# zwpku/colvars-finder

Measured on AMD Instinct MI355X. Metric: MD frames/sec through EigenFunctionTask train step, higher is better.
Workload: dtype f32

## Files before the change

colvars-finder_amd/csrc/ef16_front.hip:

```cpp
#include "ef16_common.hpp"
#include "cvf_p2p.hpp"

namespace {
template <int H, int NH, int NIT, bool ALLAL>
__global__ __launch_bounds__(1024, 4) void ef16_front_kernel(cvf_mlp_desc mlp, const float* __restrict__ theta,
                                                             const float* __restrict__ packed, cvf_pp_desc pp,
                                                             const float* __restrict__ x, int64_t B,
                                                             const float* __restrict__ a, const float* __restrict__ w,
                                                             float* __restrict__ feat_tiled, float* __restrict__ y_tiled,
                                                             float* __restrict__ saved, float* __restrict__ q_tiled,
                                                             float* __restrict__ e_tiled, double* __restrict__ partial, int launch,
                                                             const float* __restrict__ x_lag, int64_t units_x,
                                                             const float* __restrict__ w_lag) {
  constexpr int RT = Hid<H>::RT, NG = Hid<H>::NG, SMAX = 18, CTMAX = 5;
  constexpr bool kTransfer = NIT == 0;
  extern __shared__ __attribute__((aligned(16))) float lds_all[];
  const int upb = launch & 0xff;
  const int k = mlp.n_nets, D = mlp.dims[0];
  const int wave_b = __builtin_amdgcn_readfirstlane((int)threadIdx.x >> 6);
  const int usub = upb > 1 ? wave_b / k : 0;
  const int wave = wave_b - usub * k;
  const int tid = (int)threadIdx.x - usub * (64 * k), lane_in = tid & 63;
  const int nthreads = upb > 1 ? 64 * k : (int)blockDim.x, nw = nthreads >> 6;
  const int net = wave;
  const int64_t ublock = (int64_t)blockIdx.x * upb + usub;
  const bool paired = kTransfer && x_lag != nullptr && (launch >> 8) != 0;
  const int nc = pp.n_coord, nal = pp.n_align, N = pp.n_rec;
  const int stride = x_tile_stride(nc);
  const Front16Lds Lo = front16_lds(nc, nal, k);
  float* lds = lds_all + usub * (kTransfer ? Lo.g + 16 : Lo.total);
  const int64_t n_ublock = (kTransfer && !paired) ? 2 * units_x : units_x;
  const int64_t ub = ublock < n_ublock ? ublock : n_ublock - 1;
  const float* const x_first = x;
  const float* const w_first = w;
  auto run_pass = [&](const int pass) __attribute__((always_inline)) {
  const int lane = lane_in;
  const PackLayout L = pack_layout(H, NH, D);
  const URows pk = urows(packed + (int64_t)net * L.per_net, L.per_net, lane);
  const int S = (D + 3) >> 2, CT = (D + 15) >> 4;
  float a0[SMAX][RT];
  float bias[NH][RT][4];
  const int q_ = lane >> 4;
  auto request_layer0 = [&]() {
#pragma unroll
    for (int s = 0; s < SMAX; ++s) {
      const int se = s < S ? s : S - 1;
#pragma unroll
      for (int rt = 0; rt < RT; ++rt) a0[s][rt] = pk.ld(L.f0() + (se * RT + rt) * 64);
    }
    load_hid_const_u<H>(urows(theta + mlp.b_off[net][0], H, q_), bias[0]);
  };
  const bool lagged = x_lag != nullptr && (paired ? pass == 1 : ub >= units_x);
  const int64_t unit = (lagged && !paired) ? ub - units_x : ub;
  const int64_t tile = (unit >> 2) + (lagged ? (units_x >> 2) : 0);
  const int sub = (int)(unit & 3);
  x = lagged ? x_lag : x_first;
  w = lagged ? w_lag : w_first;
  float* xt = lds;
  float* refL = lds + Lo.ref;
  float* aL = lds + Lo.a;
  float* auxL = lds + Lo.aux;
  float* wL = (kTransfer && pass == 1) ? lds + Lo.g : lds + Lo.w;
  float* rsL = lds + Lo.rs;
  float* yL = lds + Lo.y + (kTransfer ? pass * (k * kU) : 0);
  float* eL = lds + Lo.e;
  float* featI = lds + Lo.feat;
  float* gI = lds + Lo.g + net * (kU * kImgP);
  const int f = lane >> 2, p = lane & 3;
  const int col = lane & 15, q = lane >> 4;

  CVF_STAMP(20);
  if (stride == nc && (unit + 1) * kU <= B && (reinterpret_cast<uintptr_t>(x) & 15) == 0) {
    const float4* src = reinterpret_cast<const float4*>(x + unit * (int64_t)(kU * nc));
    float4* dst = reinterpret_cast<float4*>(xt);
    const int n4 = (kU * nc) >> 2;
    for (int v = tid; v < n4; v += nthreads) dst[v] = src[v];
  } else {
    load_x_tile<6>(x, B, nc, unit, xt, tid, nthreads, kU);
  }
  for (int j = tid; j < 3 * nal + nc; j += nthreads) refL[j] = j < 3 * nal ? pp.ref_c[j] : (a != nullptr ? a[j - 3 * nal] : 0.0f);
  if (tid < kU) {
    const int64_t frame = unit * kU + tid;
    wL[tid] = (w != nullptr && frame < B) ? w[frame] : 0.0f;
  }
  if (wave != 0) request_layer0();
  __syncthreads();
  const float* my = xt + f * stride;
  CVF_STAMP(21);

  if (wave == 0) {
    double acc[15];
#pragma unroll
    for (int i = 0; i < 15; ++i) acc[i] = 0.0;
#pragma unroll 2
    for (int b = p; b < nal; b += 4) {
      const double x0 = (double)my[3 * b], x1 = (double)my[3 * b + 1], x2 = (double)my[3 * b + 2];
      const double r0 = (double)refL[3 * b], r1 = (double)refL[3 * b + 1], r2 = (double)refL[3 * b + 2];
      acc[0] += x0; acc[1] += x1; acc[2] += x2;
      acc[3] = fma(x0, r0, acc[3]); acc[4] = fma(x0, r1, acc[4]); acc[5] = fma(x0, r2, acc[5]);
      acc[6] = fma(x1, r0, acc[6]); acc[7] = fma(x1, r1, acc[7]); acc[8] = fma(x1, r2, acc[8]);
      acc[9] = fma(x2, r0, acc[9]); acc[10] = fma(x2, r1, acc[10]); acc[11] = fma(x2, r2, acc[11]);
      acc[12] += r0; acc[13] += r1; acc[14] += r2;
    }
#pragma unroll
    for (int i = 0; i < 15; ++i) acc[i] = quad_sumd16(acc[i]);
    const double inv = fast_rcp((double)nal);
    const double cd[3] = {acc[0] * inv, acc[1] * inv, acc[2] * inv};
    double Hm[3][3];
#pragma unroll
    for (int i = 0; i < 3; ++i)
#pragma unroll
      for (int j = 0; j < 3; ++j) Hm[i][j] = fma(-cd[i], acc[12 + j], acc[3 + 3 * i + j]);
    KabschOut ko;
    if constexpr (kTransfer) {
      kabsch_from_H<false>(Hm, ko);
#pragma unroll
      for (int i = 0; i < 6; ++i) ko.Kinv[i] = 0.0f;
    } else {
      kabsch_from_H<true>(Hm, ko);
    }
    const Centre c = centre_of(cd);
    const float av[kAuxP] = {ko.R[0], ko.R[1], ko.R[2], ko.R[3], ko.R[4], ko.R[5], ko.R[6], ko.R[7], ko.R[8], c.hi[0], c.hi[1], c.hi[2],
                             ko.Kinv[0], ko.Kinv[1], ko.Kinv[2], ko.Kinv[3], ko.Kinv[4], ko.Kinv[5], c.lo[0], c.lo[1], c.lo[2]};
#pragma unroll
    for (int i = 0; i < kAuxP; ++i)
      if ((i & 3) == p) auxL[f * kAuxP + i] = av[i];
    if (lane < 3) rsL[lane] = (float)(lane == 0 ? acc[12] : lane == 1 ? acc[13] : acc[14]);
    request_layer0();
  }
  lds_barrier();
  CVF_STAMP(22);

  {
    float R[9];
    const float* ar = auxL + f * kAuxP;
#pragma unroll
    for (int i = 0; i < 9; ++i) R[i] = ar[i];
    Centre c;
#pragma unroll
    for (int i = 0; i < 3; ++i) {
      c.hi[i] = ar[9 + i];
      c.lo[i] = ar[18 + i];
    }
    for (int at = p + 4 * wave; at < N; at += 4 * nw) {
      const V3 al = row_times(centred(my, at, c), R);
      float* fi = featI + f * kImgP + 3 * at;
      fi[0] = al.x;
      fi[1] = al.y;
      fi[2] = al.z;
    }
  }
  lds_barrier();
  CVF_STAMP(23);

  Vec<H, 1> h[NH];
  auto set_bias = [&](Vec<H, 1>& X, const float (&b)[RT][4]) {
#pragma unroll
    for (int rt = 0; rt < RT; ++rt)
#pragma unroll
      for (int r = 0; r < 4; ++r) X.v[rt][0][r] = b[rt][r];
  };
  set_bias(h[0], bias[0]);
  {
    float bf[SMAX];
    const float* fr = featI + col * kImgP;
#pragma unroll
    for (int s = 0; s < SMAX; ++s) {
      const int kf = 4 * (s < S ? s : S - 1) + q;
      bf[s] = fr[kf < D ? kf : D - 1];
    }
    HFrag<H> hf[NH > 1 ? NH - 1 : 1];
#pragma unroll
    for (int l = 1; l < NH; ++l) {
      load_hfrag_u<H>(hf[l - 1], pk, L.fh(l));
      load_hid_const_u<H>(urows(theta + mlp.b_off[net][l], H, q), bias[l]);
    }
#pragma unroll
    for (int s = 0; s < SMAX; ++s) {
      if (s < S) {
#pragma unroll
        for (int rt = 0; rt < RT; ++rt) h[0].v[rt][0] = mfma4(a0[s][rt], bf[s], h[0].v[rt][0]);
      }
    }
    CVF_STAMP(24);
    tanh_inplace<H, 1>(h[0]);
#pragma unroll
    for (int l = 1; l < NH; ++l) {
      set_bias(h[l], bias[l]);
      hidden_mul<H, 1>(h[l], hf[l - 1], h[l - 1]);
      tanh_inplace<H, 1>(h[l]);
    }
  }
  float wl[RT][4];
  load_hid_const_u<H>(urows(theta + mlp.w_off[net][NH], H, q), wl);
  const float bL = theta[mlp.b_off[net][NH]];
  HFrag<H> tf[NH > 1 ? NH - 1 : 1];
#pragma unroll
  for (int l = 1; l < NH; ++l) load_hfrag_u<H>(tf[l - 1], pk, L.th(l));

  const URows sv = urows(saved + (tile * k + net) * (int64_t)(kHand<NH>() * NG * 256) + sub * 64, kHand<NH>() * NG * 256 - sub * 64, lane);
  {
    float part = 0.0f;
#pragma unroll
    for (int rt = 0; rt < RT; ++rt)
#pragma unroll
      for (int r = 0; r < 4; ++r) part = fmaf(wl[rt][r], h[NH - 1].v[rt][0][r], part);
    const float yv = sum_over_q(part) + bL;
    yL[net * kU + col] = yv;
    y_tiled[(tile * k + net) * CVF_TILE + kU * sub + col] = yv;
  }
  CVF_STAMP(25);
  if constexpr (kTransfer) {
#pragma unroll
    for (int l = 0; l < NH; ++l)
#pragma unroll
      for (int g = 0; g < NG; ++g) sv.st((l * NG + g) * 256, h[l].v[g >> 2][0][g & 3]);
    float* ft = feat_tiled + tile * (int64_t)D * CVF_TILE + kU * sub + f;
    const float* fi = featI + f * kImgP;
#pragma unroll 1
    for (int j = p + 4 * wave; j < D; j += 4 * nw) ft[j * CVF_TILE] = fi[j];
    return;
  } else {

  {
    float t0[CTMAX][NG];
#pragma unroll
    for (int rt = 0; rt < CTMAX; ++rt)
#pragma unroll
      for (int s = 0; s < NG; ++s) t0[rt][s] = pk.ld(L.t0() + ((rt < CT ? rt : CT - 1) * NG + s) * 64);
    Vec<H, 1> d;
#pragma unroll
    for (int rt = 0; rt < RT; ++rt)
#pragma unroll
      for (int r = 0; r < 4; ++r) {
        const float hv = h[NH - 1].v[rt][0][r];
        d.v[rt][0][r] = wl[rt][r] * (1.0f - hv * hv);
      }
    Vec<H, 1> ev[NH > 1 ? NH - 1 : 1];
#pragma unroll
    for (int l = NH - 1; l >= 1; --l) {
      init_bias<H, 1>(ev[l - 1], nullptr, q);
      hidden_mul<H, 1>(ev[l - 1], tf[l - 1], d);
      tangent_of<H, 1>(d, h[l - 1], ev[l - 1]);
    }
#pragma unroll
    for (int rt = 0; rt < CTMAX; ++rt) {
      if (rt < CT) {
        f32x4 acc = {0.0f, 0.0f, 0.0f, 0.0f};
#pragma unroll
        for (int s = 0; s < NG; ++s) acc = mfma4(t0[rt][s], d.v[s >> 2][0][s & 3], acc);
        if (16 * rt + 4 * q < D) *reinterpret_cast<float4*>(gI + col * kImgP + 16 * rt + 4 * q) = float4{acc[0], acc[1], acc[2], acc[3]};
      }
    }
#pragma unroll
    for (int l = 0; l < NH; ++l)
#pragma unroll
      for (int g = 0; g < NG; ++g) sv.st((l * NG + g) * 256, h[l].v[g >> 2][0][g & 3]);
#pragma unroll
    for (int l = 1; l < NH; ++l)
#pragma unroll
      for (int g = 0; g < NG; ++g) sv.st(((NH + l - 1) * NG + g) * 256, ev[l - 1].v[g >> 2][0][g & 3]);
  }
  CVF_STAMP(26);
  asm volatile("s_waitcnt lgkmcnt(0)" ::: "memory");

  float f0b[SMAX][RT];
  {
    float R[9];
    const float* ar = auxL + f * kAuxP;
#pragma unroll
    for (int i = 0; i < 9; ++i) R[i] = ar[i];
    const Centre c = centre_of(ar[9], ar[10], ar[11]);
    float* Ul = gI + f * kImgP;
    V3 gv[NIT];
    V3 gsum = v3(0.0f, 0.0f, 0.0f);
    Outer3 Mo = {{{0.0f, 0.0f}, {0.0f, 0.0f}, {0.0f, 0.0f}}, {0.0f, 0.0f, 0.0f}};
#pragma unroll
    for (int it = 0; it < NIT; ++it) {
      int at = p + 4 * it;
      asm volatile("" : "+v"(at));
      const bool last = it == NIT - 1;
      const int ac = (last && at >= N) ? N - 1 : at;
      const float lv = (last && at >= N) ? 0.0f : 1.0f;
      gv[it] = v3(Ul[3 * ac], Ul[3 * ac + 1], Ul[3 * ac + 2]);
      const V3 gm = last ? lv * gv[it] : gv[it];
      gsum = gsum + gm;
      outer_acc(Mo, centred(my, ac, c), gm);
    }
    CVF_STAMP(27);
    gsum = v3(quad_sumf16(gsum.x), quad_sumf16(gsum.y), quad_sumf16(gsum.z));
    const V3 sump = mat_times(R, gsum);
    float M[9];
    outer_to_array(Mo, M);
#pragma unroll
    for (int i = 0; i < 9; ++i) M[i] = quad_sumf16(M[i]);
    float T[9], Z[9];
#pragma unroll
    for (int i = 0; i < 3; ++i)
#pragma unroll
      for (int j = 0; j < 3; ++j) T[3 * i + j] = R[i] * M[j] + R[3 + i] * M[3 + j] + R[6 + i] * M[6 + j];
    float Kinv[6];
#pragma unroll
    for (int i = 0; i < 6; ++i) Kinv[i] = ar[12 + i];
    const V3 s = sym_times(Kinv, v3(T[7] - T[5], T[2] - T[6], T[3] - T[1]));
#pragma unroll
    for (int i = 0; i < 3; ++i) {
      Z[3 * i + 0] = R[3 * i + 1] * s.z - R[3 * i + 2] * s.y;
      Z[3 * i + 1] = -R[3 * i + 0] * s.z + R[3 * i + 2] * s.x;
      Z[3 * i + 2] = R[3 * i + 0] * s.y - R[3 * i + 1] * s.x;
    }
    const float inv_nal = 1.0f / (float)nal;
    const V3 shift = inv_nal * sump;
    const MatCols Rc = mat_cols(R), Zc = mat_cols(Z);
    f2 E2 = {0.0f, 0.0f};
    float Ez = 0.0f;
    f2 usum_xy = {0.0f, 0.0f};
    float usum_z = 0.0f;
    Outer3 dHo = {{{0.0f, 0.0f}, {0.0f, 0.0f}, {0.0f, 0.0f}}, {0.0f, 0.0f, 0.0f}};
#pragma unroll
    for (int it = 0; it < NIT; ++it) {
      int at = p + 4 * it;
      asm volatile("" : "+v"(at));
      const bool last = it == NIT - 1;
      const int ac = (last && at >= N) ? N - 1 : at;
      const float lv = (last && at >= N) ? 0.0f : 1.0f;
      const float ma = ALLAL ? 1.0f : (ac < nal ? 1.0f : 0.0f);
      const int ar_ = ALLAL ? ac : (ac < nal ? ac : 0);
      V3 rf = v3(refL[3 * ar_], refL[3 * ar_ + 1], refL[3 * ar_ + 2]);
      if (!ALLAL) rf = ma * rf;
      f2 Gxy = ALLAL ? f2{-shift.x, -shift.y} : f2{-ma * shift.x, -ma * shift.y};
      float Gz = ALLAL ? -shift.z : -ma * shift.z;
      mat_times_acc(Rc, gv[it], Gxy, Gz);
      mat_times_acc(Zc, rf, Gxy, Gz);
      const f2 uxy = f2{aL[3 * ac], aL[3 * ac + 1]} * Gxy;
      const float uz = aL[3 * ac + 2] * Gz;
      gv[it] = v3(uxy.x, uxy.y, uz);
      const bool masked = last || !ALLAL;
      const float m = ma * lv;
      const f2 uxm = masked ? m * uxy : uxy;
      const float uzm = masked ? m * uz : uz;
      E2 = fma2(last ? lv * uxy : uxy, Gxy, E2);
      Ez = fmaf(last ? lv * uz : uz, Gz, Ez);
      usum_xy += uxm; usum_z += uzm;
      outer_acc(dHo, v3(uxm.x, uxm.y, uzm), rf);
    }
    CVF_STAMP(28);
    const float E = quad_sumf16((E2.x + E2.y) + Ez);
    const V3 usum = v3(quad_sumf16(usum_xy.x), quad_sumf16(usum_xy.y), quad_sumf16(usum_z));
    const V3 rsum = v3(rsL[0], rsL[1], rsL[2]);
    float dH[9];
    outer_to_array(dHo, dH);
#pragma unroll
    for (int i = 0; i < 9; ++i) dH[i] = quad_sumf16(dH[i]);
    eL[net * kU + f] = E;
    e_tiled[(tile * k + net) * CVF_TILE + kU * sub + f] = E;
    const V3 ubar = inv_nal * usum;
    dH[0] -= ubar.x * rsum.x; dH[1] -= ubar.x * rsum.y; dH[2] -= ubar.x * rsum.z;
    dH[3] -= ubar.y * rsum.x; dH[4] -= ubar.y * rsum.y; dH[5] -= ubar.y * rsum.z;
    dH[6] -= ubar.z * rsum.x; dH[7] -= ubar.z * rsum.y; dH[8] -= ubar.z * rsum.z;
#pragma unroll
    for (int i = 0; i < 3; ++i)
#pragma unroll
      for (int j = 0; j < 3; ++j) T[3 * i + j] = R[i] * dH[j] + R[3 + i] * dH[3 + j] + R[6 + i] * dH[6 + j];
    asm volatile("" ::: "memory");
#pragma unroll
    for (int i = 0; i < 6; ++i) Kinv[i] = ar[12 + i];
    const V3 om = sym_times(Kinv, v3(T[7] - T[5], T[2] - T[6], T[3] - T[1]));
    float dR[9];
#pragma unroll
    for (int i = 0; i < 3; ++i) {
      dR[3 * i + 0] = R[3 * i + 1] * om.z - R[3 * i + 2] * om.y;
      dR[3 * i + 1] = -R[3 * i + 0] * om.z + R[3 * i + 2] * om.x;
      dR[3 * i + 2] = R[3 * i + 0] * om.y - R[3 * i + 1] * om.x;
    }
    CVF_STAMP(31);
    const MatRows Rr = mat_rows(R), dRr = mat_rows(dR);
#pragma unroll
    for (int it = 0; it < NIT; ++it) {
      int at = p + 4 * it;
      asm volatile("" : "+v"(at));
      const int ac = (it == NIT - 1 && at >= N) ? N - 1 : at;
      f2 qxy = {0.0f, 0.0f};
      float qz = 0.0f;
      row_times_acc(Rr, gv[it] - ubar, qxy, qz);
      row_times_acc(dRr, centred(my, ac, c), qxy, qz);
      gv[it] = v3(qxy.x, qxy.y, qz);
      Ul[3 * ac] = qxy.x;
      Ul[3 * ac + 1] = qxy.y;
      Ul[3 * ac + 2] = qz;
    }
    CVF_STAMP(32);
    asm volatile("" ::: "memory");
#pragma unroll
    for (int s_ = 0; s_ < SMAX; ++s_) {
      const int se = s_ < S ? s_ : S - 1;
#pragma unroll
      for (int rt = 0; rt < RT; ++rt) f0b[s_][rt] = pk.ld(L.f0() + (se * RT + rt) * 64);
    }
    {
      asm volatile("s_waitcnt lgkmcnt(0)" ::: "memory");
      Vec<H, 1> sv0;
      init_bias<H, 1>(sv0, nullptr, q);
      const float* qr = gI + col * kImgP;
#pragma unroll
      for (int s = 0; s < SMAX; ++s) {
        if (s < S) {
          const int kf = 4 * s + q;
          const float b = qr[kf < D ? kf : D - 1];
#pragma unroll
          for (int rt = 0; rt < RT; ++rt) sv0.v[rt][0] = mfma4(f0b[s][rt], b, sv0.v[rt][0]);
        }
      }
#pragma unroll
      for (int g = 0; g < NG; ++g) sv.st(((2 * NH - 1) * NG + g) * 256, sv0.v[g >> 2][0][g & 3]);
    }
    CVF_STAMP(33);
    float* qt = q_tiled + (tile * k + net) * (int64_t)D * CVF_TILE + kU * sub + f;
#pragma unroll
    for (int it = 0; it < NIT; ++it) {
      int at = p + 4 * it;
      asm volatile("" : "+v"(at));
      const int ac = (it == NIT - 1 && at >= N) ? N - 1 : at;
      qt[(3 * ac) * CVF_TILE] = gv[it].x;
      qt[(3 * ac + 1) * CVF_TILE] = gv[it].y;
      qt[(3 * ac + 2) * CVF_TILE] = gv[it].z;
    }
  }
  CVF_STAMP(34);
  {
    float* ft = feat_tiled + tile * (int64_t)D * CVF_TILE + kU * sub + f;
    const float* fi = featI + f * kImgP;
#pragma unroll 1
    for (int j = p + 4 * wave; j < D; j += 4 * nw) ft[j * CVF_TILE] = fi[j];
  }
  CVF_STAMP(29);
  if (partial == nullptr) return;
  lds_barrier();

  if (wave == 0) {
    typedef double f64x4 __attribute__((ext_vector_type(4)));
    const int np = CVF_NPAIR(k);
    const int i = lane & 15, kq = lane >> 4;
    f64x4 d1 = {0.0, 0.0, 0.0, 0.0}, d2 = {0.0, 0.0, 0.0, 0.0};
    const float* yrow = yL + (i >= 1 && i <= k ? i - 1 : 0) * kU;
    const float* erow = eL + (i < k ? i : 0) * kU;
#pragma unroll
    for (int s_ = 0; s_ < 4; ++s_) {
      const int fr = 4 * s_ + kq;
      const double wb = (double)wL[fr];
      const double yv = (double)yrow[fr];
      const double a1 = i == 0 ? 1.0 : (i <= k ? yv : 0.0);
      const double b = i == 0 ? wb : (i <= k ? wb * yv : 0.0);
      const double a2 = i < k ? (double)erow[fr] : 0.0;
      d1 = __builtin_amdgcn_mfma_f64_16x16x4f64(a1, b, d1, 0, 0, 0);
      d2 = __builtin_amdgcn_mfma_f64_16x16x4f64(a2, b, d2, 0, 0, 0);
    }
    const int cj = lane & 15;
    const int64_t G = units_x;
#pragma unroll
    for (int r = 0; r < 4; ++r) {
      const int ri = (lane >> 4) + 4 * r;
      int t = -1;
      if (ri == 0 && cj <= k) t = cj;
      else if (ri >= 1 && ri <= cj && cj <= k) {
        const int a_ = ri - 1, b_ = cj - 1;
        t = 1 + k + a_ * k - (a_ * (a_ - 1)) / 2 + (b_ - a_);
      }
      if (t >= 0) partial[t * G + unit] = d1[r];
      if (cj == 0 && ri < k) partial[(1 + k + np + ri) * G + unit] = d2[r];
    }
  }
  CVF_STAMP(30);
  }
  };
  run_pass(0);
  if constexpr (kTransfer) {
    if (!paired) return;
    run_pass(1);
    if (partial == nullptr) return;
    const int lane = lane_in;
    const int64_t unit = ub;
    lds_barrier();
    if (wave == 0) {
      typedef double f64x4 __attribute__((ext_vector_type(4)));
      const int np = CVF_NPAIR(k);
      const int i = lane & 15, kq = lane >> 4;
      const float* y0 = lds + Lo.y;
      const float* y1 = y0 + k * kU;
      const float* w0 = lds + Lo.w;
      const float* w1 = lds + Lo.g;
      f64x4 d1 = {0.0, 0.0, 0.0, 0.0}, d2 = {0.0, 0.0, 0.0, 0.0}, d3 = {0.0, 0.0, 0.0, 0.0};
      const int yi = (i >= 1 && i <= k ? i - 1 : 0) * kU, ti = (i < k ? i : 0) * kU;
#pragma unroll
      for (int s_ = 0; s_ < 4; ++s_) {
        const int fr = 4 * s_ + kq;
        const double wb = (double)w0[fr], wl_ = (double)w1[fr];
        const double yv = (double)y0[yi + fr], ylv = (double)y1[yi + fr];
        const double a1 = i == 0 ? 1.0 : (i <= k ? yv : 0.0), b1 = i == 0 ? wb : (i <= k ? wb * yv : 0.0);
        const double a2 = i == 0 ? 1.0 : (i <= k ? ylv : 0.0), b2 = i == 0 ? wl_ : (i <= k ? wl_ * ylv : 0.0);
        const double df = i < k ? (double)y1[ti + fr] - (double)y0[ti + fr] : 0.0;
        d1 = __builtin_amdgcn_mfma_f64_16x16x4f64(a1, b1, d1, 0, 0, 0);
        d2 = __builtin_amdgcn_mfma_f64_16x16x4f64(a2, b2, d2, 0, 0, 0);
        d3 = __builtin_amdgcn_mfma_f64_16x16x4f64(df, wb * df, d3, 0, 0, 0);
      }
      const int cj = lane & 15, o = 1 + k + np;
      const int64_t G = units_x;
#pragma unroll
      for (int r = 0; r < 4; ++r) {
        const int ri = (lane >> 4) + 4 * r;
        int t = -1;
        if (ri == 0 && cj <= k) t = cj;
        else if (ri >= 1 && ri <= cj && cj <= k) {
          const int a_ = ri - 1, b_ = cj - 1;
          t = 1 + k + a_ * k - (a_ * (a_ - 1)) / 2 + (b_ - a_);
        }
        if (t >= 0) partial[t * G + unit] = d1[r];
        if (ri == 0 && cj <= k) partial[(o + cj) * G + unit] = d2[r];
        if (ri >= 1 && ri == cj && cj <= k) partial[(o + 1 + k + (cj - 1)) * G + unit] = d2[r];
        if (ri == cj && cj < k) partial[(o + 1 + 2 * k + cj) * G + unit] = d3[r];
      }
    }
  }
}
}


int cvf_ef_stats_finish_impl(const cvf_ef_cfg* cfg, int n_rows, int stat_major, const double* partial, double* stats,
                             double* loss_vec, double* coef, hipStream_t s);
int cvf_ef_stats_finish_ll(const cvf_ef_cfg* cfg, int n_rows, int stat_major, const double* partial, double* stats,
                           double* loss_vec, double* coef, hipStream_t s, const P2PLL* ll);

static int ef16_units_per_wg(int64_t units, int k, size_t lds_unit_bytes) {
  int cap = 16 / k;
  if (cap > 5) cap = 5;
  while (cap > 1 && (size_t)cap * lds_unit_bytes > 150 * 1024) --cap;
  if (cap < 1) cap = 1;
  int upb = 1;
  (void)units;
  if (const char* e = getenv("CVF_EF16_UPB")) {
    const int v = atoi(e);
    if (v >= 1 && v <= cap) upb = v;
  }
  return upb;
}

extern "C" int cvf_ef16_supported(const cvf_mlp_desc* mlp, const cvf_pp_desc* pp) {
  int H, NH;
  if (!mlp || !pp || !ef16_shape(mlp, &H, &NH) || getenv("CVF_NO_EF16")) return 0;
  if (!ef16_dispatch(H, NH, [](auto, auto) {})) return 0;
  const int fast = CVF_PP_ALIGN_CONTIG | CVF_PP_PURE_POSITION;
  if (pp->mode != CVF_PP_ALIGN || pp->align_w || (pp->flags & fast) != fast || pp->n_align > pp->n_rec || pp->n_align < 3) return 0;
  if (pp->d_r != 3 * pp->n_rec || pp->d_r != mlp->dims[0] || pp->d_r > 72 || pp->n_coord > 192 || pp->n_coord < pp->d_r) return 0;
  if (mlp->n_nets < 1 || mlp->n_nets > CVF_MAX_NETS) return 0;
  return (size_t)front16_lds(pp->n_coord, pp->n_align, mlp->n_nets).total * sizeof(float) <= 64 * 1024;
}

extern "C" int64_t cvf_ef16_scratch_doubles(int64_t B, int k) {
  const int64_t units = 4 * cvf_ntiles(B);
  const int64_t rows = units <= kMaxRows16 ? units : 0;
  return rows * cvf_ef_nstats(k, 1) + cvf_ef_stats_scratch_doubles(k, 1);
}

extern "C" int64_t cvf_ef16_rows(int64_t B) {
  const int64_t units = 4 * cvf_ntiles(B);
  return units <= kMaxRows16 ? units : 0;
}
extern "C" int cvf_ef16_finish(const cvf_ef_cfg* cfg, int64_t B, const double* scratch, double* stats, double* loss_vec, double* coef,
                               void* stream) {
  CVF_REQUIRE(cfg && scratch && stats && cvf_ef16_rows(B) > 0, "cvf_ef16_finish: bad argument");
  CVF_REQUIRE(loss_vec == nullptr || coef != nullptr, "cvf_ef16_finish: loss_vec without coef");
  return cvf_ef_stats_finish_impl(cfg, (int)cvf_ef16_rows(B), 1, scratch, stats, loss_vec, coef, (hipStream_t)stream);
}

extern "C" int cvf_ef16_finish_dp(const cvf_ef_cfg* cfg, int64_t B, const double* scratch, double* stats, double* loss_vec, double* coef,
                                  void* p2p_comm, void* stream) {
  CVF_REQUIRE(cfg && scratch && stats && loss_vec && coef && cvf_ef16_rows(B) > 0, "cvf_ef16_finish_dp: bad argument");
  const P2PLL* ll = cvf_p2p_ll(p2p_comm, 0);
  if (ll == nullptr) return -1;
  return cvf_ef_stats_finish_ll(cfg, (int)cvf_ef16_rows(B), 1, scratch, stats, loss_vec, coef, (hipStream_t)stream, ll);
}

extern "C" int64_t cvf_ef16_saved_floats(const cvf_mlp_desc* mlp, int64_t n_tiles) {
  int H, NH;
  if (!mlp || !ef16_shape(mlp, &H, &NH)) return 0;
  return n_tiles * mlp->n_nets * (2 * NH) * (int64_t)((H + 3) / 4) * 256;
}

extern "C" int cvf_ef16_front(const cvf_mlp_desc* mlp, const float* theta, const float* packed, float* feat_tiled,
                              const cvf_pp_desc* pp, const float* x, int64_t B, const float* a, float* y_tiled, float* saved,
                              float* q_tiled, float* e_tiled, const cvf_ef_cfg* cfg, const float* w, double* scratch, double* stats,
                              double* loss_vec, double* coef, void* stream) {
  CVF_REQUIRE(pp && pp->mode != CVF_PP_FACTORED, "cvf_ef16_front: takes coordinates, not CVF_PP_FACTORED records");
  CVF_REQUIRE(cvf_ef16_supported(mlp, pp), "cvf_ef16_front: shape not covered (cvf_ef16_supported() == 0)");
  CVF_REQUIRE(theta && packed && feat_tiled && x && a && y_tiled && saved && q_tiled && e_tiled && cfg && w && scratch && B > 0,
              "cvf_ef16_front: bad argument");
  CVF_REQUIRE(stats != nullptr || cvf_ef16_rows(B) > 0, "cvf_ef16_front: stats == NULL (rows left for cvf_ef16_finish) needs cvf_ef16_rows(B) > 0");
  CVF_REQUIRE(cfg->k == mlp->n_nets && cfg->lag_idx == 0, "cvf_ef16_front: generator mode only, cfg.k must equal the number of nets");
  CVF_REQUIRE(loss_vec == nullptr || coef != nullptr, "cvf_ef16_front: loss_vec without coef");
  int H, NH;
  ef16_shape(mlp, &H, &NH);
  const int k = mlp->n_nets;
  const int64_t T = cvf_ntiles(B), units = 4 * T;
  const int ns = cvf_ef_nstats(k, 0);
  const bool rows = units <= kMaxRows16;
  const size_t lds1 = (size_t)front16_lds(pp->n_coord, pp->n_align, k).total * sizeof(float);
  const int upb = ef16_units_per_wg(units, k, lds1);
  const size_t lds = lds1 * upb;
  (void)ns;
  ef16_dispatch(H, NH, [&](auto h_, auto nh_) {
    constexpr int kH = decltype(h_)::value, kNH = decltype(nh_)::value;
    auto go = [&](auto kernel) {
      if (lds > 48 * 1024) (void)hipFuncSetAttribute((const void*)kernel, hipFuncAttributeMaxDynamicSharedMemorySize, (int)lds);
      hipLaunchKernelGGL(kernel, dim3((unsigned)((units + upb - 1) / upb)), dim3(64 * k * upb), lds, (hipStream_t)stream, *mlp, theta, packed, *pp,
                         x, B, a, w, feat_tiled, y_tiled, saved, q_tiled, e_tiled, rows ? scratch : nullptr, upb, (const float*)nullptr, units,
                         (const float*)nullptr);
    };
    const int nit = (pp->n_rec + 3) / 4;
    const bool allal = pp->n_align == pp->n_rec;
#define EF16_GO(NIT_)                                                  \
    case NIT_:                                                          \
      if (allal) go(ef16_front_kernel<kH, kNH, NIT_, true>);            \
      else go(ef16_front_kernel<kH, kNH, NIT_, false>);                 \
      break;
    switch (nit) {
#ifndef CVF_DEV_SHAPES
      EF16_GO(1) EF16_GO(2) EF16_GO(3) EF16_GO(4) EF16_GO(5)
#endif
      default:
        if (allal) go(ef16_front_kernel<kH, kNH, 6, true>);
#ifndef CVF_DEV_SHAPES
        else go(ef16_front_kernel<kH, kNH, 6, false>);
#endif
    }
#undef EF16_GO
  });
  int rc = cvf_check_launch("ef16_front_kernel");
  if (rc || stats == nullptr) return rc;
  if (rows) return cvf_ef_stats_finish_impl(cfg, (int)units, 1, scratch, stats, loss_vec, coef, (hipStream_t)stream);
  return cvf_ef_stats(cfg, B, w, y_tiled, e_tiled, nullptr, nullptr, scratch, stats, loss_vec, coef, stream);
}


static int ef16_front_transfer_impl(const cvf_mlp_desc* mlp, const float* theta, const float* packed, float* feat_tiled,
                                    const cvf_pp_desc* pp, const float* x, const float* x_lag, int64_t B, float* y_tiled, float* saved,
                                    const float* w, const float* w_lag, double* rows_out, void* stream, const char* what) {
  CVF_REQUIRE(pp && pp->mode != CVF_PP_FACTORED, "%s: takes coordinates, not CVF_PP_FACTORED records", what);
  CVF_REQUIRE(cvf_ef16_supported(mlp, pp), "%s: shape not covered (cvf_ef16_supported() == 0)", what);
  CVF_REQUIRE(theta && packed && feat_tiled && x && x_lag && y_tiled && saved && B > 0, "%s: bad argument", what);
  int H, NH;
  ef16_shape(mlp, &H, &NH);
  const int k = mlp->n_nets;
  const int64_t T = cvf_ntiles(B), units = 4 * T;
  CVF_REQUIRE(2 * units < (int64_t)1 << 31, "%s: batch too large for one launch", what);
  const bool paired = rows_out != nullptr || getenv("CVF_EF16_UNPAIRED") == nullptr;
  const size_t lds1 = ((size_t)front16_lds(pp->n_coord, pp->n_align, k).g + 16) * sizeof(float);
  const int upb = paired ? ef16_units_per_wg(units, k, lds1) : 1;
  const size_t lds = lds1 * upb;
  ef16_dispatch(H, NH, [&](auto h_, auto nh_) {
    constexpr int kH = decltype(h_)::value, kNH = decltype(nh_)::value;
    auto kernel = ef16_front_kernel<kH, kNH, 0, true>;
    if (lds > 48 * 1024) (void)hipFuncSetAttribute((const void*)kernel, hipFuncAttributeMaxDynamicSharedMemorySize, (int)lds);
    hipLaunchKernelGGL(kernel, dim3((unsigned)(paired ? (units + upb - 1) / upb : 2 * units)), dim3(64 * k * upb), lds, (hipStream_t)stream, *mlp,
                       theta, packed, *pp, x, B, (const float*)nullptr, w, feat_tiled, y_tiled, saved, (float*)nullptr, (float*)nullptr,
                       rows_out, upb | (paired ? 256 : 0), x_lag, units, w_lag);
  });
  return cvf_check_launch("ef16_front_kernel");
}

extern "C" int cvf_ef16_front_transfer(const cvf_mlp_desc* mlp, const float* theta, const float* packed, float* feat_tiled,
                                       const cvf_pp_desc* pp, const float* x, const float* x_lag, int64_t B, float* y_tiled,
                                       float* saved, void* stream) {
  return ef16_front_transfer_impl(mlp, theta, packed, feat_tiled, pp, x, x_lag, B, y_tiled, saved, nullptr, nullptr, nullptr, stream,
                                  "cvf_ef16_front_transfer");
}

extern "C" int64_t cvf_ef16_transfer_rows(int64_t B, int k) { return k >= 1 ? cvf_ef16_rows(B) : 0; }
extern "C" int cvf_ef16_front_transfer_rows(const cvf_mlp_desc* mlp, const float* theta, const float* packed, float* feat_tiled,
                                            const cvf_pp_desc* pp, const float* x, const float* x_lag, int64_t B, float* y_tiled,
                                            float* saved, const float* w, const float* w_lag, double* scratch, void* stream) {
  CVF_REQUIRE(w && w_lag && scratch && mlp && cvf_ef16_transfer_rows(B, mlp->n_nets) > 0, "cvf_ef16_front_transfer_rows: bad argument");
  return ef16_front_transfer_impl(mlp, theta, packed, feat_tiled, pp, x, x_lag, B, y_tiled, saved, w, w_lag, scratch, stream,
                                  "cvf_ef16_front_transfer_rows");
}
```

Baseline: 295.4 million.

## Solve Kabsch rotation via quaternion characteristic polynomial Newton iteration

Adds a quaternion-based Kabsch solver that builds the 4x4 symmetric key matrix, finds its largest eigenvalue by a fixed count of Newton steps on the characteristic polynomial, and takes the eigenvector from an adjugate column. The non-transfer path of the front kernel now uses it in place of the previous SVD-style kabsch_from_H. The aim is a shorter, branch-light double-precision rotation solve per frame. It falls back to the old solver when the Newton step has not converged or the adjugate column is degenerate, which adds a divergent slow path and extra register pressure.

```diff
diff --git a/colvars-finder_amd/csrc/cvf_kabsch_quat.hpp b/colvars-finder_amd/csrc/cvf_kabsch_quat.hpp
--- /dev/null
+++ b/colvars-finder_amd/csrc/cvf_kabsch_quat.hpp
@@ -0,0 +1,113 @@
+#pragma once
+#include "cvf_kabsch.hpp"
+
+constexpr int kQuatNewton = 8;
+constexpr double kQuatMinCol = 1e-4;
+constexpr double kQuatMaxStep = 1e-9;
+
+CVF_HD double sym4_adj(const double (&a)[10], double (&adj)[10]) {
+  const double a00 = a[0], a01 = a[1], a02 = a[2], a03 = a[3], a11 = a[4], a12 = a[5], a13 = a[6], a22 = a[7], a23 = a[8], a33 = a[9];
+  const double s0 = a00 * a11 - a01 * a01, s1 = a00 * a12 - a01 * a02, s2 = a00 * a13 - a01 * a03;
+  const double s3 = a01 * a12 - a11 * a02, s4 = a01 * a13 - a11 * a03, s5 = a02 * a13 - a12 * a03;
+  const double c5 = a22 * a33 - a23 * a23, c4 = a12 * a33 - a13 * a23, c3 = a12 * a23 - a13 * a22;
+  const double c2 = a02 * a33 - a03 * a23, c1 = a02 * a23 - a03 * a22, c0 = a02 * a13 - a03 * a12;
+  adj[0] = a11 * c5 - a12 * c4 + a13 * c3;
+  adj[1] = -a01 * c5 + a02 * c4 - a03 * c3;
+  adj[2] = a13 * s5 - a23 * s4 + a33 * s3;
+  adj[3] = -a12 * s5 + a22 * s4 - a23 * s3;
+  adj[4] = a00 * c5 - a02 * c2 + a03 * c1;
+  adj[5] = -a03 * s5 + a23 * s2 - a33 * s1;
+  adj[6] = a02 * s5 - a22 * s2 + a23 * s1;
+  adj[7] = a03 * s4 - a13 * s2 + a33 * s0;
+  adj[8] = -a02 * s4 + a12 * s2 - a23 * s0;
+  adj[9] = a02 * s3 - a12 * s1 + a22 * s0;
+  return s0 * c5 - s1 * c4 + s2 * c3 + s3 * c2 - s4 * c1 + s5 * c0;
+}
+
+template <bool KINV = true>
+CVF_HD bool kabsch_quat(const double (&H)[3][3], KabschOut& out) {
+  double f2 = 0.0;
+#pragma unroll
+  for (int i = 0; i < 3; ++i)
+#pragma unroll
+    for (int j = 0; j < 3; ++j) f2 = fma(H[i][j], H[i][j], f2);
+  const bool nonzero = f2 > 1e-300;
+  const double sc = nonzero ? cvf_rsq(f2) : 0.0;
+  double h[3][3];
+#pragma unroll
+  for (int i = 0; i < 3; ++i)
+#pragma unroll
+    for (int j = 0; j < 3; ++j) h[i][j] = H[i][j] * sc;
+  double n[10];
+  n[0] = h[0][0] + h[1][1] + h[2][2];
+  n[1] = h[2][1] - h[1][2];
+  n[2] = h[0][2] - h[2][0];
+  n[3] = h[1][0] - h[0][1];
+  n[4] = h[0][0] - h[1][1] - h[2][2];
+  n[5] = h[0][1] + h[1][0];
+  n[6] = h[0][2] + h[2][0];
+  n[7] = -h[0][0] + h[1][1] - h[2][2];
+  n[8] = h[1][2] + h[2][1];
+  n[9] = -h[0][0] - h[1][1] + h[2][2];
+  double adj[10];
+  const double c0 = sym4_adj(n, adj);
+  const double deth = h[0][0] * (h[1][1] * h[2][2] - h[1][2] * h[2][1]) - h[0][1] * (h[1][0] * h[2][2] - h[1][2] * h[2][0]) +
+                      h[0][2] * (h[1][0] * h[2][1] - h[1][1] * h[2][0]);
+  const double c1 = -8.0 * deth;
+  const double c2 = -2.0 * (f2 * sc * sc);
+  double lam = 1.7320508075688774;
+  double step = 0.0;
+#pragma unroll
+  for (int it = 0; it < kQuatNewton; ++it) {
+    const double l2 = lam * lam;
+    const double P = fma(fma(l2 + c2, lam, c1), lam, c0);
+    const double dP = fma(fma(4.0, l2, 2.0 * c2), lam, c1);
+    const bool live = dP > 1e-300;
+    step = live ? P * cvf_rcp(live ? dP : 1.0) : 0.0;
+    lam -= step;
+  }
+  {
+    const double a[10] = {n[0] - lam, n[1], n[2], n[3], n[4] - lam, n[5], n[6], n[7] - lam, n[8], n[9] - lam};
+    (void)sym4_adj(a, adj);
+  }
+  const double cl[4][4] = {{adj[0], adj[1], adj[2], adj[3]},
+                           {adj[1], adj[4], adj[5], adj[6]},
+                           {adj[2], adj[5], adj[7], adj[8]},
+                           {adj[3], adj[6], adj[8], adj[9]}};
+  double qv[4] = {cl[0][0], cl[0][1], cl[0][2], cl[0][3]};
+  double best = qv[0] * qv[0] + qv[1] * qv[1] + qv[2] * qv[2] + qv[3] * qv[3];
+#pragma unroll
+  for (int c = 1; c < 4; ++c) {
+    const double nc = cl[c][0] * cl[c][0] + cl[c][1] * cl[c][1] + cl[c][2] * cl[c][2] + cl[c][3] * cl[c][3];
+    const bool take = nc > best;
+    best = take ? nc : best;
+#pragma unroll
+    for (int i = 0; i < 4; ++i) qv[i] = take ? cl[c][i] : qv[i];
+  }
+  const bool ok = nonzero && best >= kQuatMinCol * kQuatMinCol && fabs(step) <= kQuatMaxStep;
+  const double qn = cvf_rsq(best > 1e-300 ? best : 1.0);
+  const double w = qv[0] * qn, x = qv[1] * qn, y = qv[2] * qn, z = qv[3] * qn;
+  double R[3][3] = {{w * w + x * x - y * y - z * z, 2.0 * (x * y - w * z), 2.0 * (x * z + w * y)},
+                    {2.0 * (x * y + w * z), w * w - x * x + y * y - z * z, 2.0 * (y * z - w * x)},
+                    {2.0 * (x * z - w * y), 2.0 * (y * z + w * x), w * w - x * x - y * y + z * z}};
+  if constexpr (KINV) {
+    double Kinv[6], om[3];
+    kabsch_newton_terms(R, H, Kinv, om);
+    const double ox = om[0], oy = om[1], oz = om[2];
+#pragma unroll
+    for (int i = 0; i < 3; ++i) {
+      const double r0 = R[i][0], r1 = R[i][1], r2 = R[i][2];
+      R[i][0] = r0 + (r1 * oz - r2 * oy);
+      R[i][1] = r1 + (r2 * ox - r0 * oz);
+      R[i][2] = r2 + (r0 * oy - r1 * ox);
+    }
+#pragma unroll
+    for (int i = 0; i < 6; ++i) out.Kinv[i] = (float)Kinv[i];
+  }
+#pragma unroll
+  for (int i = 0; i < 3; ++i)
+#pragma unroll
+    for (int j = 0; j < 3; ++j) out.R[3 * i + j] = (float)R[i][j];
+  if (__builtin_expect(!ok, 0)) kabsch_from_H<KINV>(H, out);
+  return ok;
+}
diff --git a/colvars-finder_amd/csrc/ef16_front.hip b/colvars-finder_amd/csrc/ef16_front.hip
--- a/colvars-finder_amd/csrc/ef16_front.hip
+++ b/colvars-finder_amd/csrc/ef16_front.hip
@@ -1,5 +1,6 @@
 #include "ef16_common.hpp"
 #include "cvf_p2p.hpp"
+#include "cvf_kabsch_quat.hpp"
 
 namespace {
 template <int H, int NH, int NIT, bool ALLAL>
@@ -117,7 +118,7 @@
 #pragma unroll
       for (int i = 0; i < 6; ++i) ko.Kinv[i] = 0.0f;
     } else {
-      kabsch_from_H<true>(Hm, ko);
+      (void)kabsch_quat<true>(Hm, ko);
     }
     const Centre c = centre_of(cd);
     const float av[kAuxP] = {ko.R[0], ko.R[1], ko.R[2], ko.R[3], ko.R[4], ko.R[5], ko.R[6], ko.R[7], ko.R[8], c.hi[0], c.hi[1], c.hi[2],
```

Result: no change. 297.4 million (median of 6 runs) (+0.7%).
